# cure-lab/MagicDrive

Measured on NVIDIA H100. Metric: 6-view 224x400 denoising-steps/sec, higher is better.
Workload: dtype bf16

## Files before the change

magicdrive_b200/csrc/capi_gemm.cu:

```cuda
#include <cuda.h>
#include <cuda_runtime.h>
#include <stdio.h>
#include <string.h>

#include <algorithm>
#include <mutex>

#include "../../include/magicdrive_b200.h"
#define MDB_NEED_TENSORMAP
#include "common_host.h"
#include "gemm_wgmma.cuh"

using namespace mdb;

namespace {

bool make_im2col_map(CUtensorMap* m, const void* ptr, int c, int ld, const mdb_gemm_desc* d) {
  EncodeIm2colFn enc = get_encode_im2col();
  if (!enc) return false;
  const int n = d->n_img, h = d->h_in, w = d->w_in;
  cuuint64_t dims[4] = {(cuuint64_t)c, (cuuint64_t)w, (cuuint64_t)h, (cuuint64_t)n};
  cuuint64_t strides[3] = {(cuuint64_t)ld * 2, (cuuint64_t)w * ld * 2, (cuuint64_t)h * w * ld * 2};
  int lower[2] = {-d->pad_w, -d->pad_h};
  int upper[2] = {d->pad_w - (d->taps_w - 1), d->pad_h - (d->taps_h - 1)};
// ... 19 lines not shown

bool make_act_map(CUtensorMap* m, const void* ptr, int c, int ld, const mdb_gemm_desc* d, bool im2col) {
  return im2col ? make_im2col_map(m, ptr, c, ld, d)
                : make_rows_map(m, ptr, c, ld, (long long)d->n_img * d->h_out * d->w_out);
}

bool make_w_map(CUtensorMap* m, const void* ptr, int n_out, int k, int block_n) {
  EncodeTiledFn enc = get_encode();
  if (!enc) return false;
  cuuint64_t dims[2] = {(cuuint64_t)k, (cuuint64_t)n_out};
  cuuint64_t strides[1] = {(cuuint64_t)k * 2};
  cuuint32_t box[2] = {64u, (cuuint32_t)block_n};
  cuuint32_t estr[2] = {1u, 1u};
  CUresult r = enc(m, CU_TENSOR_MAP_DATA_TYPE_BFLOAT16, 2, const_cast<void*>(ptr), dims, strides, box, estr,
                   CU_TENSOR_MAP_INTERLEAVE_NONE, CU_TENSOR_MAP_SWIZZLE_128B, CU_TENSOR_MAP_L2_PROMOTION_L2_256B,
                   CU_TENSOR_MAP_FLOAT_OOB_FILL_NONE);
  return r == CUDA_SUCCESS;
}

struct Plan {
  int m_tiles;
  int ctas, m_groups;
  int block_n, n_tiles, splits, kb_per_split, kb_total;
};

int num_sms() {
  static int sms = 0;
  if (!sms) {
    int dev = 0;
    cudaGetDevice(&dev);
    if (cudaDeviceGetAttribute(&sms, cudaDevAttrMultiProcessorCount, dev) != cudaSuccess || sms <= 0) sms = 132;
  }
  return sms;
}

int validate(const mdb_gemm_desc* d) {
  if (!d || !d->a0 || !d->w || !d->out) return set_error(MDB_ERR_INVALID, "mdb_gemm_conv: null pointer");
  if (d->c0 <= 0 || d->c0 % 64 || d->c1 < 0 || d->c1 % 64)
    return set_error(MDB_ERR_UNSUPPORTED, "mdb_gemm_conv: channel counts must be multiples of 64 (c0=%d c1=%d)", d->c0,
                     d->c1);
  if (d->c1 > 0 && !d->a1) return set_error(MDB_ERR_INVALID, "mdb_gemm_conv: c1>0 but a1 is null");
  if (d->lda0 % 8 || (d->c1 > 0 && d->lda1 % 8) || d->ldo % 8 || (d->residual && d->ldr % 8))
    return set_error(MDB_ERR_UNSUPPORTED, "mdb_gemm_conv: leading dimensions must be multiples of 8");
  if (d->n_out % 8) return set_error(MDB_ERR_UNSUPPORTED, "mdb_gemm_conv: n_out must be a multiple of 8");
  if (d->stride != 1 && d->stride != 2) return set_error(MDB_ERR_UNSUPPORTED, "mdb_gemm_conv: stride must be 1 or 2");
  if (d->kernel_variant != 0 && (d->kernel_variant < 2 || d->kernel_variant > 4))
    return set_error(MDB_ERR_INVALID, "mdb_gemm_conv: kernel_variant must be 0, 2, 3 or 4");
  if (d->n_img <= 0 || d->h_out <= 0 || d->w_out <= 0 || d->taps_h <= 0 || d->taps_w <= 0)
    return set_error(MDB_ERR_INVALID, "mdb_gemm_conv: bad shape");
  if ((reinterpret_cast<uintptr_t>(d->a0) | reinterpret_cast<uintptr_t>(d->a1) | reinterpret_cast<uintptr_t>(d->w) |
       reinterpret_cast<uintptr_t>(d->out) | reinterpret_cast<uintptr_t>(d->residual)) & 15)
    return set_error(MDB_ERR_INVALID, "mdb_gemm_conv: pointers must be 16-byte aligned");
  if (d->epi_mode == 1 && (d->n_out % 256 || d->residual || d->rowbias || d->out_is_f32 || d->stats_out))
    return set_error(MDB_ERR_UNSUPPORTED, "mdb_gemm_conv: GEGLU epilogue needs n_out %% 256 == 0 and a plain bf16 output "
                                          "(no residual, per-image shift or row statistics)");
  return MDB_OK;
}

void plan_for(const mdb_gemm_desc* d, int ctas, bool allow_split, Plan* pl) {
  const int m_tiles = (int)(((long long)d->n_img * d->h_out * d->w_out + kBlockM - 1) / kBlockM);
  pl->m_tiles = m_tiles;
  pl->ctas = ctas;
  pl->m_groups = (m_tiles + ctas - 1) / ctas;
  pl->kb_total = d->taps_h * d->taps_w * ((d->c0 + d->c1) / 64);
  const int sms = num_sms();
  const int clusters = sms / ctas;
  int bn_choice = 0;
  if (d->epi_mode == 1) {
    bn_choice = 256;
  } else if (d->force_block_n) {
    bn_choice = d->force_block_n;
  } else {
    const int cands[4] = {256, 160, 128, 64};
    double best = 1e30;
    for (int i = 0; i < 4; ++i) {
      const int bn = cands[i];
      if (bn == 64 && d->n_out >= 128) continue;
      const int nt = (d->n_out + bn - 1) / bn;
      const long long groups = (long long)pl->m_groups * nt;
      const long long waves = (groups + clusters - 1) / clusters;
      const double cost = (double)waves * (bn < 96 ? 96 : bn) * 1.0 + (double)waves * 6.0;
      if (cost < best - 1e-9) best = cost, bn_choice = bn;
    }
  }
  pl->block_n = bn_choice;
  pl->n_tiles = (d->n_out + bn_choice - 1) / bn_choice;
  int splits = 1;
  const long long ctas_total = (long long)m_tiles * pl->n_tiles;
  if (!allow_split) {
    splits = 1;
  } else if (d->force_splits > 0) {
    splits = d->force_splits;
  } else if (d->epi_mode == 0 && !d->ln_stats && !d->stats_out && d->workspace && ctas_total * 2 <= sms && pl->kb_total >= 16) {
    splits = (int)(sms / ctas_total);
    if (splits > pl->kb_total / 8) splits = pl->kb_total / 8;
    if (splits > 16) splits = 16;
    if (splits < 1) splits = 1;
  }
  if (splits > pl->kb_total) splits = pl->kb_total;
  if (splits > 1) {
    const size_t need = (size_t)splits * d->n_img * d->h_out * d->w_out * d->n_out * sizeof(float);
    if (!d->workspace || d->workspace_bytes < need || d->epi_mode != 0 || d->ln_stats || d->stats_out) splits = 1;
  }
  pl->kb_per_split = (pl->kb_total + splits - 1) / splits;
  pl->splits = (pl->kb_total + pl->kb_per_split - 1) / pl->kb_per_split;
}

void make_plan(const mdb_gemm_desc* d, Plan* pl) {
  if (d->kernel_variant == 3) return plan_for(d, 2, false, pl);
  plan_for(d, 1, d->kernel_variant != 4, pl);
}

template <int BN, int CTAS>
int launch(const CUtensorMap& tA0, const CUtensorMap& tA1, const CUtensorMap& tB, const GemmParams& gp, cudaStream_t st) {
  using Cfg = WgGemmCfg<BN, CTAS>;
  static bool attr_set = false;
  if (!attr_set) {
    cudaError_t e = cudaFuncSetAttribute(gemm_wgmma_kernel<BN, CTAS>, cudaFuncAttributeMaxDynamicSharedMemorySize, Cfg::kSmemBytes);
    if (e != cudaSuccess) return set_error(MDB_ERR_CUDA, "cudaFuncSetAttribute: %s", cudaGetErrorString(e));
    attr_set = true;
  }
  const long long total = (long long)gp.m_groups * gp.n_tiles * gp.splits;
  const int clusters_max = num_sms() / CTAS;
  const int clusters = (int)(total < clusters_max ? total : clusters_max);
  cudaLaunchConfig_t cfg = {};
  cfg.gridDim = dim3(clusters * CTAS);
  cfg.blockDim = dim3(Cfg::kThreads);
  cfg.dynamicSmemBytes = Cfg::kSmemBytes;
  cfg.stream = st;
  cudaLaunchAttribute attr[2];
  attr[0].id = cudaLaunchAttributeClusterDimension;
  attr[0].val.clusterDim.x = CTAS;
  attr[0].val.clusterDim.y = 1;
  attr[0].val.clusterDim.z = 1;
  add_pdl_attr(cfg, attr, 1);
  cudaError_t e = cudaLaunchKernelEx(&cfg, gemm_wgmma_kernel<BN, CTAS>, tA0, tA1, tB, gp);
  if (e == cudaSuccess) e = cudaGetLastError();
  if (e != cudaSuccess) return set_error(MDB_ERR_CUDA, "gemm_wgmma_kernel<%d,%d> launch: %s", BN, CTAS, cudaGetErrorString(e));
  return MDB_OK;
}

template <int CTAS>
int launch_bn(int block_n, const CUtensorMap& tA0, const CUtensorMap& tA1, const CUtensorMap& tB, const GemmParams& gp,
              cudaStream_t st) {
  switch (block_n) {
    case 256: return launch<256, CTAS>(tA0, tA1, tB, gp, st);
    case 160: return launch<160, CTAS>(tA0, tA1, tB, gp, st);
    case 128: return launch<128, CTAS>(tA0, tA1, tB, gp, st);
    case 64: return launch<64, CTAS>(tA0, tA1, tB, gp, st);
    default: return set_error(MDB_ERR_UNSUPPORTED, "mdb_gemm_conv: unsupported block_n %d", block_n);
  }
}

}

extern "C" int mdb_gemm_conv_launches(const mdb_gemm_desc* d) {
  if (validate(d) != MDB_OK) return MDB_ERR_INVALID;
  Plan pl;
  make_plan(d, &pl);
  return pl.splits > 1 ? 2 : 1;
}

extern "C" int mdb_gemm_conv_stats_parts(const mdb_gemm_desc* d) {
  if (validate(d) != MDB_OK) return MDB_ERR_INVALID;
  Plan pl;
  make_plan(d, &pl);
  return pl.n_tiles;
}

extern "C" int mdb_gemm_conv_plan(const mdb_gemm_desc* d, int* plan) {
  if (validate(d) != MDB_OK) return MDB_ERR_INVALID;
  Plan pl;
  make_plan(d, &pl);
  const long long walk = (long long)pl.m_groups * pl.n_tiles * pl.splits;
  const int clusters = num_sms() / pl.ctas;
  plan[0] = pl.block_n;
  plan[1] = pl.m_tiles;
  plan[2] = pl.n_tiles;
  plan[3] = pl.splits;
  plan[4] = (int)((walk + clusters - 1) / clusters);
  return MDB_OK;
}

extern "C" int mdb_gemm_conv(const mdb_gemm_desc* d, void* stream) {
  int rc = validate(d);
  if (rc != MDB_OK) return rc;
  if (d->ln_stats && (d->taps_h != 1 || d->taps_w != 1 || !d->ln_colsum || d->ln_parts <= 0))
    return set_error(MDB_ERR_INVALID, "mdb_gemm_conv: a folded LayerNorm needs a 1x1 GEMM, ln_colsum and ln_parts");
  Plan pl;
  make_plan(d, &pl);
  if (d->epi_mode == 1 && pl.block_n != 256) return set_error(MDB_ERR_UNSUPPORTED, "GEGLU needs block_n 256");
  cudaStream_t st = static_cast<cudaStream_t>(stream);

  const bool im2col = d->taps_h != 1 || d->taps_w != 1 || d->stride != 1 || d->pad_h || d->pad_w ||
                      d->h_in != d->h_out || d->w_in != d->w_out;
  CUtensorMap tA0, tA1, tB;
  if (!make_act_map(&tA0, d->a0, d->c0, d->lda0, d, im2col))
    return set_error(MDB_ERR_CUDA, "cuTensorMapEncode%s(A0) failed (c=%d ld=%d n=%d h=%d w=%d taps=%dx%d pad=%dx%d s=%d)",
                     im2col ? "Im2col" : "Tiled", d->c0, d->lda0, d->n_img, d->h_in, d->w_in, d->taps_h, d->taps_w,
                     d->pad_h, d->pad_w, d->stride);
  if (d->c1 > 0) {
    if (!make_act_map(&tA1, d->a1, d->c1, d->lda1, d, im2col))
      return set_error(MDB_ERR_CUDA, "cuTensorMapEncode%s(A1) failed", im2col ? "Im2col" : "Tiled");
// ... 3 lines not shown
  const int ktot = d->taps_h * d->taps_w * (d->c0 + d->c1);
  if (!make_w_map(&tB, d->w, d->n_out, ktot, pl.block_n / pl.ctas))
    return set_error(MDB_ERR_CUDA, "cuTensorMapEncodeTiled(W) failed (n=%d k=%d)", d->n_out, ktot);

  GemmParams gp;
  memset(&gp, 0, sizeof(gp));
  gp.n_img = d->n_img, gp.h_out = d->h_out, gp.w_out = d->w_out, gp.n_out = d->n_out;
  gp.taps_h = d->taps_h, gp.taps_w = d->taps_w, gp.stride = d->stride, gp.pad_h = d->pad_h, gp.pad_w = d->pad_w;
  gp.cblocks0 = d->c0 / 64, gp.cblocks1 = d->c1 / 64;
  gp.im2col = im2col;
  gp.m_tiles = pl.m_tiles, gp.n_tiles = pl.n_tiles, gp.splits = pl.splits;
  gp.m_groups = pl.m_groups;
  gp.kb_per_split = pl.kb_per_split;
  gp.epi_mode = pl.splits > 1 ? EPI_PARTIAL_F32 : d->epi_mode;
  gp.out_is_f32 = d->out_is_f32;
  gp.bias = d->bias, gp.rowbias = d->rowbias, gp.rowbias_ld = d->rowbias_ld;
  gp.residual = static_cast<const __nv_bfloat16*>(d->residual), gp.ldr = d->ldr;
  gp.out = d->out, gp.ldo = d->ldo, gp.out_scale = d->out_scale;
  gp.partial = static_cast<float*>(d->workspace);
  gp.ln_stats = d->ln_stats, gp.ln_parts = d->ln_parts, gp.ln_eps = d->ln_eps, gp.ln_colsum = d->ln_colsum;
  gp.ln_inv_c = 1.0f / (float)(d->c0 + d->c1);
  gp.stats_out = d->stats_out;

  rc = pl.ctas == 2 ? launch_bn<2>(pl.block_n, tA0, tA1, tB, gp, st) : launch_bn<1>(pl.block_n, tA0, tA1, tB, gp, st);
  if (rc != MDB_OK) return rc;
  if (pl.splits > 1) {
    const long long pixels = (long long)d->n_img * d->h_out * d->w_out;
    const long long total4 = pixels * d->n_out / 4;
    const int threads = 256;
    const int blocks = (int)((total4 + threads - 1) / threads);
    cudaError_t e = launch_pdl(splitk_finalize_kernel, dim3(blocks), dim3(threads), 0, st,
                               static_cast<const float*>(d->workspace), pl.splits, pixels, d->n_out, d->h_out * d->w_out,
                               d->bias, d->rowbias, d->rowbias_ld, static_cast<const __nv_bfloat16*>(d->residual), d->ldr,
                               d->out, d->ldo, d->out_is_f32, d->out_scale);
    if (e == cudaSuccess) e = cudaGetLastError();
    if (e != cudaSuccess) return set_error(MDB_ERR_CUDA, "splitk_finalize launch: %s", cudaGetErrorString(e));
  }
  return MDB_OK;
}
```

magicdrive_b200/csrc/gemm_wgmma.cuh:

```cuda
#pragma once
#include "common_host.h"
#include "gemm_tc.cuh"
#include "ptx_cluster.cuh"
#include "wgmma.cuh"

namespace mdb {

template <int BLOCK_N, int CTAS>
struct WgGemmCfg {
  static constexpr int kBBytes = BLOCK_N * kBlockK * 2;
  static constexpr int kBRows = BLOCK_N / CTAS;
  static constexpr int kBPartBytes = kBRows * kBlockK * 2;
  static constexpr int kStageBytes = kABytes + kBBytes;
  static constexpr int kBarBytes = 256;
  static constexpr int kStagesFit = (232448 - 1024 - kBarBytes) / kStageBytes;
  static constexpr int kStages = kStagesFit > 8 ? 8 : kStagesFit;
  static constexpr int kSmemBytes = kStages * kStageBytes + 1024 + kBarBytes;
  static constexpr int kConsumerWarps = 8;
  static constexpr int kThreads = 32 * kConsumerWarps + 32;
  static constexpr int kAcc = BLOCK_N / 2;
  static_assert(kStages >= 3, "pipeline too shallow");
  static_assert(kBPartBytes % 1024 == 0, "B stage parts must keep the 1024-byte swizzle alignment");
};

__device__ __forceinline__ float2 ldg_f2(const float* p) { return __ldg(reinterpret_cast<const float2*>(p)); }

template <int BLOCK_N, int CTAS>
__global__ void __launch_bounds__(WgGemmCfg<BLOCK_N, CTAS>::kThreads, 1)
gemm_wgmma_kernel(const __grid_constant__ CUtensorMap tmA0, const __grid_constant__ CUtensorMap tmA1,
                  const __grid_constant__ CUtensorMap tmB, const GemmParams p) {
  using Cfg = WgGemmCfg<BLOCK_N, CTAS>;
  constexpr bool PAIR = CTAS == 2;
  constexpr int STAGES = Cfg::kStages;
  extern __shared__ uint8_t smem_raw[];
  uint8_t* smem = reinterpret_cast<uint8_t*>((reinterpret_cast<uintptr_t>(smem_raw) + 1023) & ~uintptr_t(1023));
  uint8_t* smA = smem;
  uint8_t* smB = smem + STAGES * kABytes;
  uint64_t* full_bar = reinterpret_cast<uint64_t*>(smem + STAGES * Cfg::kStageBytes);
  uint64_t* empty_bar = full_bar + STAGES;

  const int warp = threadIdx.x >> 5;
  const int lane = threadIdx.x & 31;
  const int cb_total = p.cblocks0 + p.cblocks1;
  const int kb_total = p.taps_h * p.taps_w * cb_total;
  const int total_tiles = p.m_groups * p.n_tiles * p.splits;
  const int rank = PAIR ? static_cast<int>(cluster_ctarank()) : 0;
  const int first_tile = static_cast<int>(blockIdx.x) / CTAS, tile_step = static_cast<int>(gridDim.x) / CTAS;

  if (warp == Cfg::kConsumerWarps && lane == 0) {
    prefetch_tmap(&tmA0);
    prefetch_tmap(&tmA1);
    prefetch_tmap(&tmB);
    for (int i = 0; i < STAGES; ++i) {
      mbar_init(&full_bar[i], 1);
      mbar_init(&empty_bar[i], CTAS * Cfg::kConsumerWarps);
    }
    fence_barrier_init();
  }
  if constexpr (PAIR) cluster_sync_all(); else __syncthreads();
  pdl_wait();
  pdl_launch_dependents();

  if (warp == Cfg::kConsumerWarps) {
    if (lane == 0) {
      const uint32_t tx_bytes = kABytes + Cfg::kBBytes;
      const int hw_out = p.h_out * p.w_out;
      int stage = 0;
      uint32_t phase = 0;
      for (int t = first_tile; t < total_tiles; t += tile_step) {
        const int mt = (t % p.m_groups) * CTAS + rank;
        const int rest = t / p.m_groups;
        const int nt = rest % p.n_tiles;
        const int z = rest / p.n_tiles;
        const int pix0 = mt * kBlockM;
        const int img0 = pix0 / hw_out;
        const int oh0 = (pix0 - img0 * hw_out) / p.w_out;
        const int ow0 = pix0 - img0 * hw_out - oh0 * p.w_out;
        const int wc = ow0 * p.stride - p.pad_w, hc = oh0 * p.stride - p.pad_h;
        const int n0 = nt * BLOCK_N;
        const int kb_begin = z * p.kb_per_split;
        const int kb_end = min(kb_total, kb_begin + p.kb_per_split);
        for (int kb = kb_begin; kb < kb_end; ++kb) {
          mbar_wait(&empty_bar[stage], phase ^ 1);
          const int tap = kb / cb_total;
          const int cb = kb - tap * cb_total;
          const int r = tap / p.taps_w, s = tap - r * p.taps_w;
          mbar_arrive_expect_tx(&full_bar[stage], tx_bytes);
          const CUtensorMap* tmA = cb < p.cblocks0 ? &tmA0 : &tmA1;
          const int c = (cb < p.cblocks0 ? cb : cb - p.cblocks0) * kBlockK;
          if (p.im2col)
            tma_load_im2col_4d(tmA, &full_bar[stage], smA + stage * kABytes, c, wc, hc, img0, static_cast<uint16_t>(s),
                               static_cast<uint16_t>(r));
          else
            tma_load_2d(tmA, &full_bar[stage], smA + stage * kABytes, c, pix0);
          if constexpr (PAIR)
            tma_load_2d_multicast(&tmB, &full_bar[stage], smB + stage * Cfg::kBBytes + rank * Cfg::kBPartBytes, kb * kBlockK,
                                  n0 + rank * Cfg::kBRows, 0x3);
          else
            tma_load_2d(&tmB, &full_bar[stage], smB + stage * Cfg::kBBytes, kb * kBlockK, n0);
          if (++stage == STAGES) {
            stage = 0;
            phase ^= 1;
          }
        }
      }
    }
  } else {
  const int wg = warp >> 2;
  const int q = lane & 3;
  const int row0 = 64 * wg + 16 * (warp & 3) + (lane >> 2);
  const int hw_out = p.h_out * p.w_out;
  const long long pixels_total = static_cast<long long>(p.n_img) * p.h_out * p.w_out;
  const float scale = p.out_scale;
  int stage = 0;
  uint32_t phase = 0;
  const uint32_t peer = rank ^ 1;
  auto release = [&](int s) {
    if (lane == 0) {
      mbar_arrive(&empty_bar[s]);
      if constexpr (PAIR) mbar_arrive_cluster_release(mapa_u32(smem_u32(&empty_bar[s]), peer));
    }
  };
  for (int t = first_tile; t < total_tiles; t += tile_step) {
    const int mt = (t % p.m_groups) * CTAS + rank;
    const int rest = t / p.m_groups;
    const int nt = rest % p.n_tiles;
    const int z = rest / p.n_tiles;
    const int n0 = nt * BLOCK_N;
    const int kb_begin = z * p.kb_per_split;
    const int nkb = min(kb_total, kb_begin + p.kb_per_split) - kb_begin;

    float acc[Cfg::kAcc];
#pragma unroll
    for (int i = 0; i < Cfg::kAcc; ++i) acc[i] = 0.f;
    int prev = -1;
    for (int i = 0; i < nkb; ++i) {
      mbar_wait(&full_bar[stage], phase);
      wgmma_fence();
      const uint64_t adesc = make_sw128_kmajor_desc(smem_u32(smA + stage * kABytes + wg * (64 * 128)));
      const uint64_t bdesc = make_sw128_kmajor_desc(smem_u32(smB + stage * Cfg::kBBytes));
#pragma unroll
      for (int k = 0; k < kBlockK / 16; ++k) WgmmaSS<BLOCK_N>::run(acc, adesc + 2 * k, bdesc + 2 * k, 1u);
      wgmma_commit();
      wgmma_wait<1>();
      if (prev >= 0) release(prev);
      prev = stage;
      if (++stage == STAGES) {
        stage = 0;
        phase ^= 1;
      }
    }
    wgmma_wait<0>();
    if (prev >= 0) release(prev);

    int img[2];
    long long pix[2];
    bool ok[2];
#pragma unroll
    for (int h = 0; h < 2; ++h) {
      const int px = mt * kBlockM + row0 + 8 * h;
      img[h] = px / hw_out;
      pix[h] = px;
      ok[h] = pix[h] < pixels_total;
    }
    if (p.epi_mode == EPI_PARTIAL_F32) {
#pragma unroll
      for (int j = 0; j < BLOCK_N / 8; ++j) {
        const int col = n0 + 8 * j + 2 * q;
        if (col >= p.n_out) continue;
#pragma unroll
        for (int h = 0; h < 2; ++h)
          if (ok[h])
            *reinterpret_cast<float2*>(p.partial + (static_cast<long long>(z) * pixels_total + pix[h]) * p.n_out + col) =
                make_float2(acc[4 * j + 2 * h], acc[4 * j + 2 * h + 1]);
      }
      continue;
    }
    float rowA[2] = {scale, scale}, rowB[2] = {0.f, 0.f};
    if (p.ln_stats != nullptr) {
#pragma unroll
      for (int h = 0; h < 2; ++h) {
        if (!ok[h]) continue;
        const float2* sp = reinterpret_cast<const float2*>(p.ln_stats) + pix[h] * p.ln_parts;
        float s = 0.f, ss = 0.f;
        for (int j = 0; j < p.ln_parts; ++j) {
          const float2 v = __ldg(sp + j);
          s += v.x, ss += v.y;
        }
        const float mean = s * p.ln_inv_c;
        const float rstd = rsqrtf(fmaxf(ss * p.ln_inv_c - mean * mean, 0.f) + p.ln_eps);
        rowA[h] = rstd * scale;
        rowB[h] = -mean * rowA[h];
      }
    }
    const bool has_ln = p.ln_stats != nullptr;
    if (p.epi_mode == EPI_GEGLU) {
      constexpr int HALF = BLOCK_N / 2;
      const int on0 = nt * HALF;
      __nv_bfloat16* out = static_cast<__nv_bfloat16*>(p.out);
#pragma unroll
      for (int j = 0; j < HALF / 8; ++j) {
        const int c = 8 * j + 2 * q;
        const float2 bv = p.bias ? ldg_f2(p.bias + n0 + c) : make_float2(0.f, 0.f);
        const float2 bg = p.bias ? ldg_f2(p.bias + n0 + HALF + c) : make_float2(0.f, 0.f);
        const float2 cv = has_ln ? ldg_f2(p.ln_colsum + n0 + c) : make_float2(0.f, 0.f);
        const float2 cg = has_ln ? ldg_f2(p.ln_colsum + n0 + HALF + c) : make_float2(0.f, 0.f);
#pragma unroll
        for (int h = 0; h < 2; ++h) {
          if (!ok[h]) continue;
          const float a0 = fmaf(rowA[h], acc[4 * j + 2 * h], fmaf(rowB[h], cv.x, bv.x * scale));
          const float a1 = fmaf(rowA[h], acc[4 * j + 2 * h + 1], fmaf(rowB[h], cv.y, bv.y * scale));
          const float g0 = fmaf(rowA[h], acc[4 * (j + HALF / 8) + 2 * h], fmaf(rowB[h], cg.x, bg.x * scale));
          const float g1 = fmaf(rowA[h], acc[4 * (j + HALF / 8) + 2 * h + 1], fmaf(rowB[h], cg.y, bg.y * scale));
          *reinterpret_cast<uint32_t*>(out + pix[h] * p.ldo + on0 + c) = pack_bf16(a0 * gelu_erf(g0), a1 * gelu_erf(g1));
        }
      }
      continue;
    }
    float st_s[2] = {0.f, 0.f}, st_ss[2] = {0.f, 0.f};
#pragma unroll
    for (int j = 0; j < BLOCK_N / 8; ++j) {
      const int col = n0 + 8 * j + 2 * q;
      if (col >= p.n_out) continue;
      const float2 b = p.bias ? ldg_f2(p.bias + col) : make_float2(0.f, 0.f);
      const float2 cs = has_ln ? ldg_f2(p.ln_colsum + col) : make_float2(0.f, 0.f);
#pragma unroll
      for (int h = 0; h < 2; ++h) {
        if (!ok[h]) continue;
        float2 cb = b;
        if (p.rowbias) {
          const float2 rb = ldg_f2(p.rowbias + static_cast<long long>(img[h]) * p.rowbias_ld + col);
          cb.x += rb.x, cb.y += rb.y;
        }
        float v0 = fmaf(rowA[h], acc[4 * j + 2 * h], fmaf(rowB[h], cs.x, cb.x * scale));
        float v1 = fmaf(rowA[h], acc[4 * j + 2 * h + 1], fmaf(rowB[h], cs.y, cb.y * scale));
        if (p.residual) {
          const float2 r = __bfloat1622float2(*reinterpret_cast<const __nv_bfloat162*>(p.residual + pix[h] * p.ldr + col));
          v0 += r.x, v1 += r.y;
        }
        st_s[h] += v0 + v1;
        st_ss[h] = fmaf(v0, v0, fmaf(v1, v1, st_ss[h]));
        if (p.out_is_f32)
          *reinterpret_cast<float2*>(static_cast<float*>(p.out) + pix[h] * p.ldo + col) = make_float2(v0, v1);
        else
          *reinterpret_cast<uint32_t*>(static_cast<__nv_bfloat16*>(p.out) + pix[h] * p.ldo + col) = pack_bf16(v0, v1);
      }
    }
    if (p.stats_out != nullptr) {
#pragma unroll
      for (int h = 0; h < 2; ++h) {
        st_s[h] += __shfl_xor_sync(0xffffffffu, st_s[h], 1);
        st_s[h] += __shfl_xor_sync(0xffffffffu, st_s[h], 2);
        st_ss[h] += __shfl_xor_sync(0xffffffffu, st_ss[h], 1);
        st_ss[h] += __shfl_xor_sync(0xffffffffu, st_ss[h], 2);
        if (q == 0 && ok[h])
          reinterpret_cast<float2*>(p.stats_out)[pix[h] * p.n_tiles + nt] = make_float2(st_s[h], st_ss[h]);
      }
    }
  }
  }
  __syncwarp();
  if constexpr (PAIR) cluster_sync_all();
}

}
```

magicdrive_b200/csrc/ptx.cuh:

```cuda
#pragma once
#include <cuda.h>
#include <cuda_bf16.h>
#include <cuda_runtime.h>
#include <stdint.h>

namespace mdb {

__device__ __forceinline__ uint32_t smem_u32(const void* p) {
  return static_cast<uint32_t>(__cvta_generic_to_shared(p));
}

__device__ __forceinline__ bool elect_one() {
  uint32_t pred = 0;
  asm volatile(
      "{\n\t"
      ".reg .pred P;\n\t"
      "elect.sync _|P, 0xffffffff;\n\t"
      "selp.b32 %0, 1, 0, P;\n\t"
      "}\n"
      : "=r"(pred));
  return pred != 0;
}

__device__ __forceinline__ void mbar_init(uint64_t* bar, uint32_t count) {
  asm volatile("mbarrier.init.shared::cta.b64 [%0], %1;" ::"r"(smem_u32(bar)), "r"(count));
}
__device__ __forceinline__ void fence_barrier_init() {
  asm volatile("fence.mbarrier_init.release.cluster;" ::: "memory");
}
__device__ __forceinline__ void fence_proxy_async() {
  asm volatile("fence.proxy.async.shared::cta;" ::: "memory");
}
__device__ __forceinline__ bool mbar_test(uint64_t* bar, uint32_t parity) {
  uint32_t ok;
  asm volatile(
      "{\n\t"
      ".reg .pred P1;\n\t"
      "mbarrier.test_wait.parity.shared::cta.b64 P1, [%1], %2;\n\t"
      "selp.u32 %0, 1, 0, P1;\n\t"
      "}\n"
      : "=r"(ok)
      : "r"(smem_u32(bar)), "r"(parity)
      : "memory");
  return ok != 0;
// ... 102 lines not shown
```

magicdrive_b200/ops.py:

```python
import ctypes as C
import contextlib
import os
from typing import Optional

import torch

from . import _lib
from ._lib import GemmDesc, check

BF16 = torch.bfloat16
F32 = torch.float32

GEMM_VARIANT = int(os.environ.get('MDB_GEMM_VARIANT', '0'))
_launches = 0
_profile = None


def start_profile():
    global _profile
    _profile = []


def stop_profile(with_info: bool = False):
    global _profile
# ... 114 lines not shown
    d.out, d.ldo, d.out_is_f32, d.out_scale = _ptr(out), ldo, int(out_f32), float(out_scale)
    d.epi_mode = 1 if geglu else 0
    if allow_split_k and not geglu:
        ws = workspace(64 << 20, a0.device)
        d.workspace, d.workspace_bytes = ws.data_ptr(), ws.numel()
    else:
        d.workspace, d.workspace_bytes = None, 0
    d.force_block_n, d.force_splits = force_block_n, force_splits
    d.kernel_variant = kernel_variant or GEMM_VARIANT
    L = _lib.lib()
    if ln is not None:
        d.ln_stats, d.ln_parts, d.ln_eps, d.ln_colsum = ln.data.data_ptr(), ln.parts, float(ln_eps), _ptr(ln_colsum)
    stats = None
    if emit_stats:
        d.stats_out = 1
        parts = L.mdb_gemm_conv_stats_parts(C.byref(d))
        if parts <= 0:
            check(parts, "mdb_gemm_conv_stats_parts")
        stats = RowStats(torch.empty((pixels, parts, 2), dtype=F32, device=a0.device), parts)
        d.stats_out = stats.data.data_ptr()
    e0 = _prof_begin()
    check(L.mdb_gemm_conv(C.byref(d), _stream()), "mdb_gemm_conv")
    if e0 is not None:
        plan = (C.c_int * 5)()
        check(L.mdb_gemm_conv_plan(C.byref(d), plan), "mdb_gemm_conv_plan")
        _prof_end("gemm_conv", 2.0 * pixels * n_out * taps * taps * (c0 + c1), e0,
                  f"M={pixels} N={n_out} K={taps * taps * (c0 + c1)} img={n_img}x{h_out}x{w_out} taps={taps} s={stride} "
                  f"geglu={int(geglu)} res={int(residual is not None)} | BN={plan[0]} tiles={plan[1]}x{plan[2]}x{plan[3]} "
                  f"waves={plan[4]}")
    _launches += L.mdb_gemm_conv_launches(C.byref(d))
    return (out, stats) if emit_stats else out


@contextlib.contextmanager
def pdl_region(enabled: bool = True):
    lib = _lib.lib()
    old = lib.mdb_set_pdl(int(enabled))
    try:
        yield
    finally:
        lib.mdb_set_pdl(old)


def linear(x: torch.Tensor, w: torch.Tensor, bias=None, residual=None, out=None, ldo=None, geglu=False,
           out_f32=False, out_scale=1.0, **kw):
    m, k = x.shape
    return gemm_conv(x, w, n_img=1, h_in=1, w_in=m, c0=k, lda0=x.stride(0), n_out=w.shape[0], bias=bias,
                     residual=residual, ldr=(residual.stride(0) if residual is not None else 0), out=out, ldo=ldo,
                     geglu=geglu, out_f32=out_f32, out_scale=out_scale, **kw)


def conv_direct(x, wgt, bias, *, n, h, w, cin, cout, k, stride=(1, 1), pad=(1, 1), silu=False, residual=None,
# ... 215 lines not shown
```

Measured before the change: 56.65.

## Add ping-pong warp-specialized WGMMA GEMM kernel with automatic schedule selection

Adds a ping-pong GEMM kernel with one producer warpgroup and two consumer warpgroups. The consumers alternate whole output tiles, ordered by named barriers, so one tile's epilogue overlaps the next tile's MMA main loop. Register budgets are rebalanced with setmaxnreg. The planner picks ping-pong by default for single-CTA plans with block_n below 256 when each CTA walks enough tiles. The epilogue is factored into a shared function and now groups residual loads ahead of use. The risk is a longer per-tile mainloop from each consumer handling the full 128-row tile, plus extra sync overhead.

```diff
diff --git a/magicdrive_b200/csrc/capi_gemm.cu b/magicdrive_b200/csrc/capi_gemm.cu
--- a/magicdrive_b200/csrc/capi_gemm.cu
+++ b/magicdrive_b200/csrc/capi_gemm.cu
@@ -65,6 +65,7 @@
   int m_tiles;
   int ctas, m_groups;
   int block_n, n_tiles, splits, kb_per_split, kb_total;
+  bool pingpong;
 };
 
 int num_sms() {
@@ -87,8 +88,8 @@
     return set_error(MDB_ERR_UNSUPPORTED, "mdb_gemm_conv: leading dimensions must be multiples of 8");
   if (d->n_out % 8) return set_error(MDB_ERR_UNSUPPORTED, "mdb_gemm_conv: n_out must be a multiple of 8");
   if (d->stride != 1 && d->stride != 2) return set_error(MDB_ERR_UNSUPPORTED, "mdb_gemm_conv: stride must be 1 or 2");
-  if (d->kernel_variant != 0 && (d->kernel_variant < 2 || d->kernel_variant > 4))
-    return set_error(MDB_ERR_INVALID, "mdb_gemm_conv: kernel_variant must be 0, 2, 3 or 4");
+  if (d->kernel_variant != 0 && (d->kernel_variant < 2 || d->kernel_variant > 6))
+    return set_error(MDB_ERR_INVALID, "mdb_gemm_conv: kernel_variant must be 0, 2, 3, 4, 5 or 6");
   if (d->n_img <= 0 || d->h_out <= 0 || d->w_out <= 0 || d->taps_h <= 0 || d->taps_w <= 0)
     return set_error(MDB_ERR_INVALID, "mdb_gemm_conv: bad shape");
   if ((reinterpret_cast<uintptr_t>(d->a0) | reinterpret_cast<uintptr_t>(d->a1) | reinterpret_cast<uintptr_t>(d->w) |
@@ -100,7 +101,16 @@
   return MDB_OK;
 }
 
-void plan_for(const mdb_gemm_desc* d, int ctas, bool allow_split, Plan* pl) {
+enum Sched { SCHED_AUTO, SCHED_COOP, SCHED_PINGPONG };
+
+bool use_pingpong(int ctas, int block_n, long long walk, int clusters, Sched sched) {
+  if (ctas != 1 || block_n == 256 || sched == SCHED_COOP) return false;
+  if (sched == SCHED_PINGPONG) return true;
+  const long long per_cta = (walk + clusters - 1) / clusters;
+  return per_cta >= 4 && (per_cta % 2 == 0 || per_cta >= 8);
+}
+
+void plan_for(const mdb_gemm_desc* d, int ctas, bool allow_split, Sched sched, Plan* pl) {
   const int m_tiles = (int)(((long long)d->n_img * d->h_out * d->w_out + kBlockM - 1) / kBlockM);
   pl->m_tiles = m_tiles;
   pl->ctas = ctas;
@@ -147,19 +157,24 @@
   }
   pl->kb_per_split = (pl->kb_total + splits - 1) / splits;
   pl->splits = (pl->kb_total + pl->kb_per_split - 1) / pl->kb_per_split;
+  pl->pingpong = use_pingpong(ctas, pl->block_n, (long long)pl->m_groups * pl->n_tiles * pl->splits, clusters, sched);
 }
 
 void make_plan(const mdb_gemm_desc* d, Plan* pl) {
-  if (d->kernel_variant == 3) return plan_for(d, 2, false, pl);
-  plan_for(d, 1, d->kernel_variant != 4, pl);
-}
-
-template <int BN, int CTAS>
+  if (d->kernel_variant == 3) return plan_for(d, 2, false, SCHED_COOP, pl);
+  const Sched sched = d->kernel_variant == 5 ? SCHED_COOP : d->kernel_variant == 6 ? SCHED_PINGPONG : SCHED_AUTO;
+  plan_for(d, 1, d->kernel_variant != 4, sched, pl);
+}
+
+template <int BN, int CTAS, bool PP>
 int launch(const CUtensorMap& tA0, const CUtensorMap& tA1, const CUtensorMap& tB, const GemmParams& gp, cudaStream_t st) {
   using Cfg = WgGemmCfg<BN, CTAS>;
+  void (*kernel)(CUtensorMap, CUtensorMap, CUtensorMap, GemmParams);
+  if constexpr (PP) kernel = gemm_wgmma_pp_kernel<BN>;
+  else kernel = gemm_wgmma_kernel<BN, CTAS>;
   static bool attr_set = false;
   if (!attr_set) {
-    cudaError_t e = cudaFuncSetAttribute(gemm_wgmma_kernel<BN, CTAS>, cudaFuncAttributeMaxDynamicSharedMemorySize, Cfg::kSmemBytes);
+    cudaError_t e = cudaFuncSetAttribute(kernel, cudaFuncAttributeMaxDynamicSharedMemorySize, Cfg::kSmemBytes);
     if (e != cudaSuccess) return set_error(MDB_ERR_CUDA, "cudaFuncSetAttribute: %s", cudaGetErrorString(e));
     attr_set = true;
   }
@@ -168,7 +183,7 @@
   const int clusters = (int)(total < clusters_max ? total : clusters_max);
   cudaLaunchConfig_t cfg = {};
   cfg.gridDim = dim3(clusters * CTAS);
-  cfg.blockDim = dim3(Cfg::kThreads);
+  cfg.blockDim = dim3(PP ? kPingPongThreads : Cfg::kThreads);
   cfg.dynamicSmemBytes = Cfg::kSmemBytes;
   cfg.stream = st;
   cudaLaunchAttribute attr[2];
@@ -177,9 +192,11 @@
   attr[0].val.clusterDim.y = 1;
   attr[0].val.clusterDim.z = 1;
   add_pdl_attr(cfg, attr, 1);
-  cudaError_t e = cudaLaunchKernelEx(&cfg, gemm_wgmma_kernel<BN, CTAS>, tA0, tA1, tB, gp);
+  cudaError_t e = cudaLaunchKernelEx(&cfg, kernel, tA0, tA1, tB, gp);
   if (e == cudaSuccess) e = cudaGetLastError();
-  if (e != cudaSuccess) return set_error(MDB_ERR_CUDA, "gemm_wgmma_kernel<%d,%d> launch: %s", BN, CTAS, cudaGetErrorString(e));
+  if (e != cudaSuccess)
+    return set_error(MDB_ERR_CUDA, "%s<%d,%d> launch: %s", PP ? "gemm_wgmma_pp_kernel" : "gemm_wgmma_kernel", BN, CTAS,
+                     cudaGetErrorString(e));
   return MDB_OK;
 }
 
@@ -187,11 +204,21 @@
 int launch_bn(int block_n, const CUtensorMap& tA0, const CUtensorMap& tA1, const CUtensorMap& tB, const GemmParams& gp,
               cudaStream_t st) {
   switch (block_n) {
-    case 256: return launch<256, CTAS>(tA0, tA1, tB, gp, st);
-    case 160: return launch<160, CTAS>(tA0, tA1, tB, gp, st);
-    case 128: return launch<128, CTAS>(tA0, tA1, tB, gp, st);
-    case 64: return launch<64, CTAS>(tA0, tA1, tB, gp, st);
+    case 256: return launch<256, CTAS, false>(tA0, tA1, tB, gp, st);
+    case 160: return launch<160, CTAS, false>(tA0, tA1, tB, gp, st);
+    case 128: return launch<128, CTAS, false>(tA0, tA1, tB, gp, st);
+    case 64: return launch<64, CTAS, false>(tA0, tA1, tB, gp, st);
     default: return set_error(MDB_ERR_UNSUPPORTED, "mdb_gemm_conv: unsupported block_n %d", block_n);
+  }
+}
+
+int launch_pingpong(int block_n, const CUtensorMap& tA0, const CUtensorMap& tA1, const CUtensorMap& tB,
+                    const GemmParams& gp, cudaStream_t st) {
+  switch (block_n) {
+    case 160: return launch<160, 1, true>(tA0, tA1, tB, gp, st);
+    case 128: return launch<128, 1, true>(tA0, tA1, tB, gp, st);
+    case 64: return launch<64, 1, true>(tA0, tA1, tB, gp, st);
+    default: return set_error(MDB_ERR_UNSUPPORTED, "mdb_gemm_conv: no ping-pong kernel for block_n %d", block_n);
   }
 }
 
@@ -222,6 +249,7 @@
   plan[2] = pl.n_tiles;
   plan[3] = pl.splits;
   plan[4] = (int)((walk + clusters - 1) / clusters);
+  plan[5] = pl.pingpong ? 1 : 0;
   return MDB_OK;
 }
 
@@ -271,7 +299,10 @@
   gp.ln_inv_c = 1.0f / (float)(d->c0 + d->c1);
   gp.stats_out = d->stats_out;
 
-  rc = pl.ctas == 2 ? launch_bn<2>(pl.block_n, tA0, tA1, tB, gp, st) : launch_bn<1>(pl.block_n, tA0, tA1, tB, gp, st);
+  if (pl.pingpong)
+    rc = launch_pingpong(pl.block_n, tA0, tA1, tB, gp, st);
+  else
+    rc = pl.ctas == 2 ? launch_bn<2>(pl.block_n, tA0, tA1, tB, gp, st) : launch_bn<1>(pl.block_n, tA0, tA1, tB, gp, st);
   if (rc != MDB_OK) return rc;
   if (pl.splits > 1) {
     const long long pixels = (long long)d->n_img * d->h_out * d->w_out;
diff --git a/magicdrive_b200/csrc/gemm_wgmma.cuh b/magicdrive_b200/csrc/gemm_wgmma.cuh
--- a/magicdrive_b200/csrc/gemm_wgmma.cuh
+++ b/magicdrive_b200/csrc/gemm_wgmma.cuh
@@ -23,7 +23,204 @@
   static_assert(kBPartBytes % 1024 == 0, "B stage parts must keep the 1024-byte swizzle alignment");
 };
 
+constexpr int kPingPongThreads = 384;
+constexpr int kPingPongProducerRegs = 40;
+constexpr int kPingPongConsumerRegs = 232;
+constexpr int kTurnBar = 1;
+
+constexpr int kEpiGroup = 2;
+
 __device__ __forceinline__ float2 ldg_f2(const float* p) { return __ldg(reinterpret_cast<const float2*>(p)); }
+
+struct TileCoord {
+  int mt, nt, z, kb_begin, nkb;
+};
+__device__ __forceinline__ TileCoord tile_coord(const GemmParams& p, int t, int kb_total, int ctas, int rank) {
+  TileCoord c;
+  c.mt = (t % p.m_groups) * ctas + rank;
+  const int rest = t / p.m_groups;
+  c.nt = rest % p.n_tiles;
+  c.z = rest / p.n_tiles;
+  c.kb_begin = c.z * p.kb_per_split;
+  c.nkb = min(kb_total, c.kb_begin + p.kb_per_split) - c.kb_begin;
+  return c;
+}
+
+template <int BLOCK_N, int CTAS>
+__device__ __forceinline__ void produce_tiles(const CUtensorMap* tmA0, const CUtensorMap* tmA1, const CUtensorMap* tmB,
+                                              const GemmParams& p, uint8_t* smA, uint8_t* smB, uint64_t* full_bar,
+                                              uint64_t* empty_bar, int rank, int first_tile, int tile_step) {
+  using Cfg = WgGemmCfg<BLOCK_N, CTAS>;
+  constexpr int STAGES = Cfg::kStages;
+  const uint32_t tx_bytes = kABytes + Cfg::kBBytes;
+  const int cb_total = p.cblocks0 + p.cblocks1;
+  const int kb_total = p.taps_h * p.taps_w * cb_total;
+  const int total_tiles = p.m_groups * p.n_tiles * p.splits;
+  const int hw_out = p.h_out * p.w_out;
+  int stage = 0;
+  uint32_t phase = 0;
+  for (int t = first_tile; t < total_tiles; t += tile_step) {
+    const TileCoord tc = tile_coord(p, t, kb_total, CTAS, rank);
+    const int pix0 = tc.mt * kBlockM;
+    const int img0 = pix0 / hw_out;
+    const int oh0 = (pix0 - img0 * hw_out) / p.w_out;
+    const int ow0 = pix0 - img0 * hw_out - oh0 * p.w_out;
+    const int wc = ow0 * p.stride - p.pad_w, hc = oh0 * p.stride - p.pad_h;
+    const int n0 = tc.nt * BLOCK_N;
+    for (int kb = tc.kb_begin; kb < tc.kb_begin + tc.nkb; ++kb) {
+      mbar_wait(&empty_bar[stage], phase ^ 1);
+      const int tap = kb / cb_total;
+      const int cb = kb - tap * cb_total;
+      const int r = tap / p.taps_w, s = tap - r * p.taps_w;
+      mbar_arrive_expect_tx(&full_bar[stage], tx_bytes);
+      const CUtensorMap* tmA = cb < p.cblocks0 ? tmA0 : tmA1;
+      const int c = (cb < p.cblocks0 ? cb : cb - p.cblocks0) * kBlockK;
+      if (p.im2col)
+        tma_load_im2col_4d(tmA, &full_bar[stage], smA + stage * kABytes, c, wc, hc, img0, static_cast<uint16_t>(s),
+                           static_cast<uint16_t>(r));
+      else
+        tma_load_2d(tmA, &full_bar[stage], smA + stage * kABytes, c, pix0);
+      if constexpr (CTAS == 2)
+        tma_load_2d_multicast(tmB, &full_bar[stage], smB + stage * Cfg::kBBytes + rank * Cfg::kBPartBytes, kb * kBlockK,
+                              n0 + rank * Cfg::kBRows, 0x3);
+      else
+        tma_load_2d(tmB, &full_bar[stage], smB + stage * Cfg::kBBytes, kb * kBlockK, n0);
+      if (++stage == STAGES) {
+        stage = 0;
+        phase ^= 1;
+      }
+    }
+  }
+}
+
+template <int BLOCK_N>
+__device__ __forceinline__ void epilogue(const float (&acc)[BLOCK_N / 2], const GemmParams& p, const TileCoord& tc, int row,
+                                         int q) {
+  const int hw_out = p.h_out * p.w_out;
+  const long long pixels_total = static_cast<long long>(p.n_img) * p.h_out * p.w_out;
+  const float scale = p.out_scale;
+  const int n0 = tc.nt * BLOCK_N;
+  int img[2];
+  long long pix[2];
+  bool ok[2];
+#pragma unroll
+  for (int h = 0; h < 2; ++h) {
+    const int px = tc.mt * kBlockM + row + 8 * h;
+    img[h] = px / hw_out;
+    pix[h] = px;
+    ok[h] = pix[h] < pixels_total;
+  }
+  if (p.epi_mode == EPI_PARTIAL_F32) {
+#pragma unroll
+    for (int j = 0; j < BLOCK_N / 8; ++j) {
+      const int col = n0 + 8 * j + 2 * q;
+      if (col >= p.n_out) continue;
+#pragma unroll
+      for (int h = 0; h < 2; ++h)
+        if (ok[h])
+          *reinterpret_cast<float2*>(p.partial + (static_cast<long long>(tc.z) * pixels_total + pix[h]) * p.n_out + col) =
+              make_float2(acc[4 * j + 2 * h], acc[4 * j + 2 * h + 1]);
+    }
+    return;
+  }
+  float rowA[2] = {scale, scale}, rowB[2] = {0.f, 0.f};
+  if (p.ln_stats != nullptr) {
+#pragma unroll
+    for (int h = 0; h < 2; ++h) {
+      if (!ok[h]) continue;
+      const float2* sp = reinterpret_cast<const float2*>(p.ln_stats) + pix[h] * p.ln_parts;
+      float s = 0.f, ss = 0.f;
+      for (int j = 0; j < p.ln_parts; ++j) {
+        const float2 v = __ldg(sp + j);
+        s += v.x, ss += v.y;
+      }
+      const float mean = s * p.ln_inv_c;
+      const float rstd = rsqrtf(fmaxf(ss * p.ln_inv_c - mean * mean, 0.f) + p.ln_eps);
+      rowA[h] = rstd * scale;
+      rowB[h] = -mean * rowA[h];
+    }
+  }
+  const bool has_ln = p.ln_stats != nullptr;
+  if (p.epi_mode == EPI_GEGLU) {
+    constexpr int HALF = BLOCK_N / 2;
+    const int on0 = tc.nt * HALF;
+    __nv_bfloat16* out = static_cast<__nv_bfloat16*>(p.out);
+#pragma unroll
+    for (int j = 0; j < HALF / 8; ++j) {
+      const int c = 8 * j + 2 * q;
+      const float2 bv = p.bias ? ldg_f2(p.bias + n0 + c) : make_float2(0.f, 0.f);
+      const float2 bg = p.bias ? ldg_f2(p.bias + n0 + HALF + c) : make_float2(0.f, 0.f);
+      const float2 cv = has_ln ? ldg_f2(p.ln_colsum + n0 + c) : make_float2(0.f, 0.f);
+      const float2 cg = has_ln ? ldg_f2(p.ln_colsum + n0 + HALF + c) : make_float2(0.f, 0.f);
+#pragma unroll
+      for (int h = 0; h < 2; ++h) {
+        if (!ok[h]) continue;
+        const float a0 = fmaf(rowA[h], acc[4 * j + 2 * h], fmaf(rowB[h], cv.x, bv.x * scale));
+        const float a1 = fmaf(rowA[h], acc[4 * j + 2 * h + 1], fmaf(rowB[h], cv.y, bv.y * scale));
+        const float g0 = fmaf(rowA[h], acc[4 * (j + HALF / 8) + 2 * h], fmaf(rowB[h], cg.x, bg.x * scale));
+        const float g1 = fmaf(rowA[h], acc[4 * (j + HALF / 8) + 2 * h + 1], fmaf(rowB[h], cg.y, bg.y * scale));
+        *reinterpret_cast<uint32_t*>(out + pix[h] * p.ldo + on0 + c) = pack_bf16(a0 * gelu_erf(g0), a1 * gelu_erf(g1));
+      }
+    }
+    return;
+  }
+  constexpr int G = BLOCK_N == 256 ? 1 : kEpiGroup;
+  static_assert((BLOCK_N / 8) % G == 0, "column groups must split evenly");
+  float st_s[2] = {0.f, 0.f}, st_ss[2] = {0.f, 0.f};
+#pragma unroll
+  for (int j0 = 0; j0 < BLOCK_N / 8; j0 += G) {
+    uint32_t res[G][2];
+#pragma unroll
+    for (int u = 0; u < G; ++u) {
+      const int col = n0 + 8 * (j0 + u) + 2 * q;
+#pragma unroll
+      for (int h = 0; h < 2; ++h)
+        res[u][h] = p.residual && col < p.n_out && ok[h]
+                        ? *reinterpret_cast<const uint32_t*>(p.residual + pix[h] * p.ldr + col)
+                        : 0u;
+    }
+#pragma unroll
+    for (int u = 0; u < G; ++u) {
+      const int j = j0 + u;
+      const int col = n0 + 8 * j + 2 * q;
+      if (col >= p.n_out) continue;
+      const float2 b = p.bias ? ldg_f2(p.bias + col) : make_float2(0.f, 0.f);
+      const float2 cs = has_ln ? ldg_f2(p.ln_colsum + col) : make_float2(0.f, 0.f);
+#pragma unroll
+      for (int h = 0; h < 2; ++h) {
+        if (!ok[h]) continue;
+        float2 cb = b;
+        if (p.rowbias) {
+          const float2 rb = ldg_f2(p.rowbias + static_cast<long long>(img[h]) * p.rowbias_ld + col);
+          cb.x += rb.x, cb.y += rb.y;
+        }
+        float v0 = fmaf(rowA[h], acc[4 * j + 2 * h], fmaf(rowB[h], cs.x, cb.x * scale));
+        float v1 = fmaf(rowA[h], acc[4 * j + 2 * h + 1], fmaf(rowB[h], cs.y, cb.y * scale));
+        if (p.residual) {
+          const float2 r = __bfloat1622float2(*reinterpret_cast<const __nv_bfloat162*>(&res[u][h]));
+          v0 += r.x, v1 += r.y;
+        }
+        st_s[h] += v0 + v1;
+        st_ss[h] = fmaf(v0, v0, fmaf(v1, v1, st_ss[h]));
+        if (p.out_is_f32)
+          *reinterpret_cast<float2*>(static_cast<float*>(p.out) + pix[h] * p.ldo + col) = make_float2(v0, v1);
+        else
+          *reinterpret_cast<uint32_t*>(static_cast<__nv_bfloat16*>(p.out) + pix[h] * p.ldo + col) = pack_bf16(v0, v1);
+      }
+    }
+  }
+  if (p.stats_out != nullptr) {
+#pragma unroll
+    for (int h = 0; h < 2; ++h) {
+      st_s[h] += __shfl_xor_sync(0xffffffffu, st_s[h], 1);
+      st_s[h] += __shfl_xor_sync(0xffffffffu, st_s[h], 2);
+      st_ss[h] += __shfl_xor_sync(0xffffffffu, st_ss[h], 1);
+      st_ss[h] += __shfl_xor_sync(0xffffffffu, st_ss[h], 2);
+      if (q == 0 && ok[h])
+        reinterpret_cast<float2*>(p.stats_out)[pix[h] * p.n_tiles + tc.nt] = make_float2(st_s[h], st_ss[h]);
+    }
+  }
+}
 
 template <int BLOCK_N, int CTAS>
 __global__ void __launch_bounds__(WgGemmCfg<BLOCK_N, CTAS>::kThreads, 1)
@@ -41,8 +238,7 @@
 
   const int warp = threadIdx.x >> 5;
   const int lane = threadIdx.x & 31;
-  const int cb_total = p.cblocks0 + p.cblocks1;
-  const int kb_total = p.taps_h * p.taps_w * cb_total;
+  const int kb_total = p.taps_h * p.taps_w * (p.cblocks0 + p.cblocks1);
   const int total_tiles = p.m_groups * p.n_tiles * p.splits;
   const int rank = PAIR ? static_cast<int>(cluster_ctarank()) : 0;
   const int first_tile = static_cast<int>(blockIdx.x) / CTAS, tile_step = static_cast<int>(gridDim.x) / CTAS;
@@ -62,56 +258,12 @@
   pdl_launch_dependents();
 
   if (warp == Cfg::kConsumerWarps) {
-    if (lane == 0) {
-      const uint32_t tx_bytes = kABytes + Cfg::kBBytes;
-      const int hw_out = p.h_out * p.w_out;
-      int stage = 0;
-      uint32_t phase = 0;
-      for (int t = first_tile; t < total_tiles; t += tile_step) {
-        const int mt = (t % p.m_groups) * CTAS + rank;
-        const int rest = t / p.m_groups;
-        const int nt = rest % p.n_tiles;
-        const int z = rest / p.n_tiles;
-        const int pix0 = mt * kBlockM;
-        const int img0 = pix0 / hw_out;
-        const int oh0 = (pix0 - img0 * hw_out) / p.w_out;
-        const int ow0 = pix0 - img0 * hw_out - oh0 * p.w_out;
-        const int wc = ow0 * p.stride - p.pad_w, hc = oh0 * p.stride - p.pad_h;
-        const int n0 = nt * BLOCK_N;
-        const int kb_begin = z * p.kb_per_split;
-        const int kb_end = min(kb_total, kb_begin + p.kb_per_split);
-        for (int kb = kb_begin; kb < kb_end; ++kb) {
-          mbar_wait(&empty_bar[stage], phase ^ 1);
-          const int tap = kb / cb_total;
-          const int cb = kb - tap * cb_total;
-          const int r = tap / p.taps_w, s = tap - r * p.taps_w;
-          mbar_arrive_expect_tx(&full_bar[stage], tx_bytes);
-          const CUtensorMap* tmA = cb < p.cblocks0 ? &tmA0 : &tmA1;
-          const int c = (cb < p.cblocks0 ? cb : cb - p.cblocks0) * kBlockK;
-          if (p.im2col)
-            tma_load_im2col_4d(tmA, &full_bar[stage], smA + stage * kABytes, c, wc, hc, img0, static_cast<uint16_t>(s),
-                               static_cast<uint16_t>(r));
-          else
-            tma_load_2d(tmA, &full_bar[stage], smA + stage * kABytes, c, pix0);
-          if constexpr (PAIR)
-            tma_load_2d_multicast(&tmB, &full_bar[stage], smB + stage * Cfg::kBBytes + rank * Cfg::kBPartBytes, kb * kBlockK,
-                                  n0 + rank * Cfg::kBRows, 0x3);
-          else
-            tma_load_2d(&tmB, &full_bar[stage], smB + stage * Cfg::kBBytes, kb * kBlockK, n0);
-          if (++stage == STAGES) {
-            stage = 0;
-            phase ^= 1;
-          }
-        }
-      }
-    }
+    if (lane == 0)
+      produce_tiles<BLOCK_N, CTAS>(&tmA0, &tmA1, &tmB, p, smA, smB, full_bar, empty_bar, rank, first_tile, tile_step);
   } else {
   const int wg = warp >> 2;
   const int q = lane & 3;
   const int row0 = 64 * wg + 16 * (warp & 3) + (lane >> 2);
-  const int hw_out = p.h_out * p.w_out;
-  const long long pixels_total = static_cast<long long>(p.n_img) * p.h_out * p.w_out;
-  const float scale = p.out_scale;
   int stage = 0;
   uint32_t phase = 0;
   const uint32_t peer = rank ^ 1;
@@ -122,19 +274,13 @@
     }
   };
   for (int t = first_tile; t < total_tiles; t += tile_step) {
-    const int mt = (t % p.m_groups) * CTAS + rank;
-    const int rest = t / p.m_groups;
-    const int nt = rest % p.n_tiles;
-    const int z = rest / p.n_tiles;
-    const int n0 = nt * BLOCK_N;
-    const int kb_begin = z * p.kb_per_split;
-    const int nkb = min(kb_total, kb_begin + p.kb_per_split) - kb_begin;
+    const TileCoord tc = tile_coord(p, t, kb_total, CTAS, rank);
 
     float acc[Cfg::kAcc];
 #pragma unroll
     for (int i = 0; i < Cfg::kAcc; ++i) acc[i] = 0.f;
     int prev = -1;
-    for (int i = 0; i < nkb; ++i) {
+    for (int i = 0; i < tc.nkb; ++i) {
       mbar_wait(&full_bar[stage], phase);
       wgmma_fence();
       const uint64_t adesc = make_sw128_kmajor_desc(smem_u32(smA + stage * kABytes + wg * (64 * 128)));
@@ -152,115 +298,102 @@
     }
     wgmma_wait<0>();
     if (prev >= 0) release(prev);
-
-    int img[2];
-    long long pix[2];
-    bool ok[2];
-#pragma unroll
-    for (int h = 0; h < 2; ++h) {
-      const int px = mt * kBlockM + row0 + 8 * h;
-      img[h] = px / hw_out;
-      pix[h] = px;
-      ok[h] = pix[h] < pixels_total;
-    }
-    if (p.epi_mode == EPI_PARTIAL_F32) {
-#pragma unroll
-      for (int j = 0; j < BLOCK_N / 8; ++j) {
-        const int col = n0 + 8 * j + 2 * q;
-        if (col >= p.n_out) continue;
-#pragma unroll
-        for (int h = 0; h < 2; ++h)
-          if (ok[h])
-            *reinterpret_cast<float2*>(p.partial + (static_cast<long long>(z) * pixels_total + pix[h]) * p.n_out + col) =
-                make_float2(acc[4 * j + 2 * h], acc[4 * j + 2 * h + 1]);
-      }
-      continue;
-    }
-    float rowA[2] = {scale, scale}, rowB[2] = {0.f, 0.f};
-    if (p.ln_stats != nullptr) {
-#pragma unroll
-      for (int h = 0; h < 2; ++h) {
-        if (!ok[h]) continue;
-        const float2* sp = reinterpret_cast<const float2*>(p.ln_stats) + pix[h] * p.ln_parts;
-        float s = 0.f, ss = 0.f;
-        for (int j = 0; j < p.ln_parts; ++j) {
-          const float2 v = __ldg(sp + j);
-          s += v.x, ss += v.y;
-        }
-        const float mean = s * p.ln_inv_c;
-        const float rstd = rsqrtf(fmaxf(ss * p.ln_inv_c - mean * mean, 0.f) + p.ln_eps);
-        rowA[h] = rstd * scale;
-        rowB[h] = -mean * rowA[h];
-      }
-    }
-    const bool has_ln = p.ln_stats != nullptr;
-    if (p.epi_mode == EPI_GEGLU) {
-      constexpr int HALF = BLOCK_N / 2;
-      const int on0 = nt * HALF;
-      __nv_bfloat16* out = static_cast<__nv_bfloat16*>(p.out);
-#pragma unroll
-      for (int j = 0; j < HALF / 8; ++j) {
-        const int c = 8 * j + 2 * q;
-        const float2 bv = p.bias ? ldg_f2(p.bias + n0 + c) : make_float2(0.f, 0.f);
-        const float2 bg = p.bias ? ldg_f2(p.bias + n0 + HALF + c) : make_float2(0.f, 0.f);
-        const float2 cv = has_ln ? ldg_f2(p.ln_colsum + n0 + c) : make_float2(0.f, 0.f);
-        const float2 cg = has_ln ? ldg_f2(p.ln_colsum + n0 + HALF + c) : make_float2(0.f, 0.f);
-#pragma unroll
-        for (int h = 0; h < 2; ++h) {
-          if (!ok[h]) continue;
-          const float a0 = fmaf(rowA[h], acc[4 * j + 2 * h], fmaf(rowB[h], cv.x, bv.x * scale));
-          const float a1 = fmaf(rowA[h], acc[4 * j + 2 * h + 1], fmaf(rowB[h], cv.y, bv.y * scale));
-          const float g0 = fmaf(rowA[h], acc[4 * (j + HALF / 8) + 2 * h], fmaf(rowB[h], cg.x, bg.x * scale));
-          const float g1 = fmaf(rowA[h], acc[4 * (j + HALF / 8) + 2 * h + 1], fmaf(rowB[h], cg.y, bg.y * scale));
-          *reinterpret_cast<uint32_t*>(out + pix[h] * p.ldo + on0 + c) = pack_bf16(a0 * gelu_erf(g0), a1 * gelu_erf(g1));
-        }
-      }
-      continue;
-    }
-    float st_s[2] = {0.f, 0.f}, st_ss[2] = {0.f, 0.f};
-#pragma unroll
-    for (int j = 0; j < BLOCK_N / 8; ++j) {
-      const int col = n0 + 8 * j + 2 * q;
-      if (col >= p.n_out) continue;
-      const float2 b = p.bias ? ldg_f2(p.bias + col) : make_float2(0.f, 0.f);
-      const float2 cs = has_ln ? ldg_f2(p.ln_colsum + col) : make_float2(0.f, 0.f);
-#pragma unroll
-      for (int h = 0; h < 2; ++h) {
-        if (!ok[h]) continue;
-        float2 cb = b;
-        if (p.rowbias) {
-          const float2 rb = ldg_f2(p.rowbias + static_cast<long long>(img[h]) * p.rowbias_ld + col);
-          cb.x += rb.x, cb.y += rb.y;
-        }
-        float v0 = fmaf(rowA[h], acc[4 * j + 2 * h], fmaf(rowB[h], cs.x, cb.x * scale));
-        float v1 = fmaf(rowA[h], acc[4 * j + 2 * h + 1], fmaf(rowB[h], cs.y, cb.y * scale));
-        if (p.residual) {
-          const float2 r = __bfloat1622float2(*reinterpret_cast<const __nv_bfloat162*>(p.residual + pix[h] * p.ldr + col));
-          v0 += r.x, v1 += r.y;
-        }
-        st_s[h] += v0 + v1;
-        st_ss[h] = fmaf(v0, v0, fmaf(v1, v1, st_ss[h]));
-        if (p.out_is_f32)
-          *reinterpret_cast<float2*>(static_cast<float*>(p.out) + pix[h] * p.ldo + col) = make_float2(v0, v1);
-        else
-          *reinterpret_cast<uint32_t*>(static_cast<__nv_bfloat16*>(p.out) + pix[h] * p.ldo + col) = pack_bf16(v0, v1);
-      }
-    }
-    if (p.stats_out != nullptr) {
-#pragma unroll
-      for (int h = 0; h < 2; ++h) {
-        st_s[h] += __shfl_xor_sync(0xffffffffu, st_s[h], 1);
-        st_s[h] += __shfl_xor_sync(0xffffffffu, st_s[h], 2);
-        st_ss[h] += __shfl_xor_sync(0xffffffffu, st_ss[h], 1);
-        st_ss[h] += __shfl_xor_sync(0xffffffffu, st_ss[h], 2);
-        if (q == 0 && ok[h])
-          reinterpret_cast<float2*>(p.stats_out)[pix[h] * p.n_tiles + nt] = make_float2(st_s[h], st_ss[h]);
-      }
-    }
+    epilogue<BLOCK_N>(acc, p, tc, row0, q);
   }
   }
   __syncwarp();
   if constexpr (PAIR) cluster_sync_all();
 }
 
-}
+template <int BLOCK_N>
+__global__ void __launch_bounds__(kPingPongThreads, 1)
+gemm_wgmma_pp_kernel(const __grid_constant__ CUtensorMap tmA0, const __grid_constant__ CUtensorMap tmA1,
+                     const __grid_constant__ CUtensorMap tmB, const GemmParams p) {
+  using Cfg = WgGemmCfg<BLOCK_N, 1>;
+  constexpr int STAGES = Cfg::kStages;
+  extern __shared__ uint8_t smem_raw[];
+  uint8_t* smem = reinterpret_cast<uint8_t*>((reinterpret_cast<uintptr_t>(smem_raw) + 1023) & ~uintptr_t(1023));
+  uint8_t* smA = smem;
+  uint8_t* smB = smem + STAGES * kABytes;
+  uint64_t* full_bar = reinterpret_cast<uint64_t*>(smem + STAGES * Cfg::kStageBytes);
+  uint64_t* empty_bar = full_bar + STAGES;
+
+  const int warp = threadIdx.x >> 5;
+  const int lane = threadIdx.x & 31;
+  const int wg = warp >> 2;
+  const int kb_total = p.taps_h * p.taps_w * (p.cblocks0 + p.cblocks1);
+  const int total_tiles = p.m_groups * p.n_tiles * p.splits;
+  const int first_tile = static_cast<int>(blockIdx.x), tile_step = static_cast<int>(gridDim.x);
+
+  if (threadIdx.x == 0) {
+    prefetch_tmap(&tmA0);
+    prefetch_tmap(&tmA1);
+    prefetch_tmap(&tmB);
+    for (int i = 0; i < STAGES; ++i) {
+      mbar_init(&full_bar[i], 1);
+      mbar_init(&empty_bar[i], 4);
+    }
+    fence_barrier_init();
+  }
+  __syncthreads();
+  pdl_wait();
+  pdl_launch_dependents();
+
+  if (wg == 0) {
+    setmaxnreg_dec<kPingPongProducerRegs>();
+    if (warp == 0 && lane == 0)
+      produce_tiles<BLOCK_N, 1>(&tmA0, &tmA1, &tmB, p, smA, smB, full_bar, empty_bar, 0, first_tile, tile_step);
+    return;
+  }
+  setmaxnreg_inc<kPingPongConsumerRegs>();
+  const int c = wg - 1;
+  const int q = lane & 3;
+  const int row0 = 16 * (warp & 3) + (lane >> 2);
+  int stage = 0;
+  uint32_t phase = 0;
+  int j = 0;
+  for (int t = first_tile; t < total_tiles; t += tile_step, ++j) {
+    const TileCoord tc = tile_coord(p, t, kb_total, 1, 0);
+    if ((j & 1) != c) {
+      stage += tc.nkb;
+      phase ^= (stage / STAGES) & 1;
+      stage %= STAGES;
+      continue;
+    }
+    if (j > 0) named_bar_sync(kTurnBar + c, 256);
+
+    float acc[2][Cfg::kAcc];
+#pragma unroll
+    for (int h = 0; h < 2; ++h)
+#pragma unroll
+      for (int i = 0; i < Cfg::kAcc; ++i) acc[h][i] = 0.f;
+    int prev = -1;
+    for (int i = 0; i < tc.nkb; ++i) {
+      mbar_wait(&full_bar[stage], phase);
+      wgmma_fence();
+      const uint64_t adesc0 = make_sw128_kmajor_desc(smem_u32(smA + stage * kABytes));
+      const uint64_t adesc1 = make_sw128_kmajor_desc(smem_u32(smA + stage * kABytes + 64 * 128));
+      const uint64_t bdesc = make_sw128_kmajor_desc(smem_u32(smB + stage * Cfg::kBBytes));
+#pragma unroll
+      for (int k = 0; k < kBlockK / 16; ++k) {
+        WgmmaSS<BLOCK_N>::run(acc[0], adesc0 + 2 * k, bdesc + 2 * k, 1u);
+        WgmmaSS<BLOCK_N>::run(acc[1], adesc1 + 2 * k, bdesc + 2 * k, 1u);
+      }
+      wgmma_commit();
+      wgmma_wait<1>();
+      if (prev >= 0 && lane == 0) mbar_arrive(&empty_bar[prev]);
+      prev = stage;
+      if (++stage == STAGES) {
+        stage = 0;
+        phase ^= 1;
+      }
+    }
+    if (t + tile_step < total_tiles) named_bar_arrive(kTurnBar + (c ^ 1), 256);
+    wgmma_wait<0>();
+    if (prev >= 0 && lane == 0) mbar_arrive(&empty_bar[prev]);
+    epilogue<BLOCK_N>(acc[0], p, tc, row0, q);
+    epilogue<BLOCK_N>(acc[1], p, tc, 64 + row0, q);
+  }
+}
+
+}
diff --git a/magicdrive_b200/csrc/ptx.cuh b/magicdrive_b200/csrc/ptx.cuh
--- a/magicdrive_b200/csrc/ptx.cuh
+++ b/magicdrive_b200/csrc/ptx.cuh
@@ -20,6 +20,21 @@
       "}\n"
       : "=r"(pred));
   return pred != 0;
+}
+
+__device__ __forceinline__ void named_bar_sync(int id, int threads) {
+  asm volatile("bar.sync %0, %1;" ::"r"(id), "r"(threads) : "memory");
+}
+__device__ __forceinline__ void named_bar_arrive(int id, int threads) {
+  asm volatile("bar.arrive %0, %1;" ::"r"(id), "r"(threads) : "memory");
+}
+template <int N>
+__device__ __forceinline__ void setmaxnreg_dec() {
+  asm volatile("setmaxnreg.dec.sync.aligned.u32 %0;" ::"n"(N));
+}
+template <int N>
+__device__ __forceinline__ void setmaxnreg_inc() {
+  asm volatile("setmaxnreg.inc.sync.aligned.u32 %0;" ::"n"(N));
 }
 
 __device__ __forceinline__ void mbar_init(uint64_t* bar, uint32_t count) {
diff --git a/magicdrive_b200/ops.py b/magicdrive_b200/ops.py
--- a/magicdrive_b200/ops.py
+++ b/magicdrive_b200/ops.py
@@ -160,12 +160,12 @@
     e0 = _prof_begin()
     check(L.mdb_gemm_conv(C.byref(d), _stream()), "mdb_gemm_conv")
     if e0 is not None:
-        plan = (C.c_int * 5)()
+        plan = (C.c_int * 6)()
         check(L.mdb_gemm_conv_plan(C.byref(d), plan), "mdb_gemm_conv_plan")
         _prof_end("gemm_conv", 2.0 * pixels * n_out * taps * taps * (c0 + c1), e0,
                   f"M={pixels} N={n_out} K={taps * taps * (c0 + c1)} img={n_img}x{h_out}x{w_out} taps={taps} s={stride} "
                   f"geglu={int(geglu)} res={int(residual is not None)} | BN={plan[0]} tiles={plan[1]}x{plan[2]}x{plan[3]} "
-                  f"waves={plan[4]}")
+                  f"waves={plan[4]} sched={'pp' if plan[5] else 'coop'}")
     _launches += L.mdb_gemm_conv_launches(C.byref(d))
     return (out, stats) if emit_stats else out
 
```

Result: faster. 59.64 (median of 6 runs) (+5.3%).
